# AnnSeidel/genometools

Hardware: AMD Instinct MI355X
Metric: Gbp/s ESA build (suf+lcp+bwt), 3 Gbp DNA, 1/2/4/8 MI355X; bit-exact vs CPU (higher is better)
Workload: dtype u64; 1 GPU; human-like DNA (2% N, 24 seqs, repeats) n=3000000000 seed=43 -suf -lcp -bwt (BASELINE.json configs[2]); parallelism=1 device, pair_suffixes=341032298, tied_suffixes=390540711, refine_rounds=9, maxbranchdepth=8256

## Files before the change

### genometools_amd/csrc/esa_engine.hip

```cpp
#include <stdarg.h>
#include <stdlib.h>
#include <chrono>
#include <type_traits>
#include <utility>
#include <vector>
#include "../../include/gtamd_esa.h"
#include "esa_prims.h"
#include "esa_devutil.h"
#include "esa_own.h"

static thread_local char g_err[1024] = "";
void gtamd_set_error(const char *fmt, ...) {
  va_list ap;
  va_start(ap, fmt);
  vsnprintf(g_err, sizeof g_err, fmt, ap);
  va_end(ap);
}
extern "C" const char *gtamd_esa_last_error(void) { return g_err; }

extern "C" int gtamd_device_count(void) {
  GTAMD_ABI_BEGIN
  int n = 0;
  if (hipGetDeviceCount(&n) != hipSuccess) return 0;
  return n;
// ... 1532 lines not shown
      xfirst[y][x] = (r & PAIR_SWAP) != 0;
    }
    u64 pos[4];
    int who[4] = {0, 0, 0, 0};
    for (int k = 0; k < g; k++) pos[k] = sa[i + k];
    for (int k = 0; k < g; k++) {
      int place = 0;
      for (int o = 0; o < g; o++)
        if (o != k && xfirst[o][k]) place++;
      who[place] = k;
    }
    u32 perm = 0;
    for (int k = 0; k < g; k++) {
      sa[i + k] = (P) pos[who[k]];
      perm |= (u32) who[k] << (2 * k);
      if (k > 0) {
        const u32 lv = lc[who[k - 1]][who[k]];
        slcp[3 * j + (k - 1)] = lv;
        sum += lv;
        nlarge += lv >= GTAMD_LCPOVERFLOW;
        mx = lv > mx ? lv : mx;
      }
    }
    sres[j] = perm | ((u32) g << 8);
    for (int k = 1; k < g; k++) {
      const u64 e = i + k;
      atomicAnd(reinterpret_cast<unsigned long long *>(&tiebits2[e >> 6]), ~(1ull << (e & 63)));
    }
    done = (u32) g;
  }
#pragma unroll
  for (int d = 32; d >= 1; d >>= 1) {
    sum += __shfl_xor(sum, d, 64);
    nlarge += __shfl_xor(nlarge, d, 64);
    done += __shfl_xor(done, d, 64);
    const u32 o = __shfl_xor(mx, d, 64);
    mx = o > mx ? o : mx;
  }
  if (lane == 0) { s_sum[w] = sum; s_large[w] = nlarge; s_max[w] = mx; s_cnt[w] = done; }
  __syncthreads();
  if (threadIdx.x == 0) {
    unsigned long long S = 0, Lg = 0;
    u32 M = 0, D = 0;
    for (int x = 0; x < 4; x++) {
      S += s_sum[x]; Lg += s_large[x]; D += s_cnt[x]; M = s_max[x] > M ? s_max[x] : M;
    }
    if (S) atomicAdd(&stats->lcpsum, S);
    if (Lg) atomicAdd(&stats->numlarge, Lg);
    if (M) atomicMax(&stats->maxlcp, M);
    if (D) atomicAdd(&stats->smalldone, (unsigned long long) D);
  }
}

template <typename P>
__global__ __launch_bounds__(256) void k_small_apply(
    const u32 *__restrict__ sidx, const u32 *__restrict__ sres, const u32 *__restrict__ slcp,
    u64 ns, const P *__restrict__ sa, u64 *__restrict__ suf, u8 *__restrict__ lcp,
    u8 *__restrict__ bwt, u32 *__restrict__ lcpfull, u64 index_offset, Stats *stats) {
  for (u64 j = (u64) blockIdx.x * 256 + threadIdx.x; j < ns; j += (u64) gridDim.x * 256) {
    const u32 r = sres[j];
    const u64 i = sidx[j];
    const int g = (int) (r >> 8) & 7;
    u8 old[4] = {0, 0, 0, 0};
    if (bwt != nullptr)
      for (int k = 0; k < g; k++) old[k] = bwt[i + k];
    for (int k = 0; k < g; k++) {
      const u64 p = sa[i + k];
      if (suf != nullptr) suf[i + k] = p;
      if (bwt != nullptr) bwt[i + k] = old[(r >> (2 * k)) & 3u];
      if (p == 0) stats->longest = index_offset + i + k;
      if (k > 0 && lcp != nullptr) {
        const u32 lv = slcp[3 * j + (k - 1)];
        lcp[i + k] = (u8) (lv < GTAMD_LCPOVERFLOW ? lv : GTAMD_LCPOVERFLOW);
        if (lv >= GTAMD_LCPOVERFLOW) lcpfull[i + k] = lv;
      }
    }
  }
}

constexpr int PE_STAGE = 2048;
template <typename P>
__global__ __launch_bounds__(256) void k_pair_emit(
    const u64 *__restrict__ tiebits, u64 nwords, const u32 *__restrict__ off,
    const P *__restrict__ sa, P *__restrict__ pkey, u64 *__restrict__ pval,
    u32 *__restrict__ pidx) {
  __shared__ u32 s_scan[4];
  __shared__ P s_pk[PE_STAGE];
  __shared__ u64 s_pv[PE_STAGE];
  __shared__ u32 s_pi[PE_STAGE];
  const u64 w = (u64) blockIdx.x * 256 + threadIdx.x;
  u64 ph = 0;
  if (w < nwords) {
    const u64 t = tiebits[w];
    const u64 nx = w + 1 < nwords ? tiebits[w + 1] : 0ull;
    ph = pair_heads(t, nx);
  }
  u32 tot;
  u32 local = block_scan_excl_sum((u32) __popcll(ph), &tot, s_scan);
  const u32 base = off[blockIdx.x];
  const bool staged = tot <= (u32) PE_STAGE;
  while (ph) {
    const int b = __ffsll((unsigned long long) ph) - 1;
    ph &= ph - 1;
    const u64 i = w * 64 + b;
    const u64 j = (u64) base + local;
    const P a = sa[i];
    const u64 v = (sizeof(P) == 4 ? (u64) sa[i + 1] : i) | (j << 32);
    if (staged) { s_pk[local] = a; s_pv[local] = v; s_pi[local] = (u32) i; }
    else { pkey[j] = a; pval[j] = v; pidx[j] = (u32) i; }
    local++;
  }
  if (!staged) return;
  __syncthreads();
  for (u32 k = threadIdx.x; k < tot; k += 256) {
    pkey[base + k] = s_pk[k];
    pval[base + k] = s_pv[k];
    pidx[base + k] = s_pi[k];
  }
}

constexpr int PR_LINE = 16;
template <int BITS, typename P>
__global__ __launch_bounds__(256) void k_pair_resolve(
    Text t, const P *__restrict__ pkey, const u64 *__restrict__ pval, u64 nrec, u64 np,
    const P *__restrict__ sa, u32 *__restrict__ res, Stats *stats, int chunk) {
  __shared__ unsigned long long s_sum[4], s_large[4];
  __shared__ u32 s_max[4];
  const int lane = threadIdx.x & 63, w = threadIdx.x >> 6;
  unsigned long long sum = 0, nlarge = 0;
  u32 mx = 0;
  const u64 nchunks = (nrec + chunk - 1) / chunk;
  for (u64 c = (u64) blockIdx.x * 256 + threadIdx.x; c < nchunks;
       c += (u64) gridDim.x * 256) {
    constexpr int RING = 4;
    u64 ra[RING] = {0, 0, 0, 0}, rb[RING] = {0, 0, 0, 0}, rl[RING] = {0, 0, 0, 0};
    bool rf[RING] = {true, true, true, true};
    int filled = 0;
    for (int e0 = 0; e0 < chunk; e0 += PR_LINE) {
      const u64 s0 = c * chunk + e0;
      if (s0 >= nrec) break;
      P ak[PR_LINE];
      u64 ivk[PR_LINE];
      if (s0 + PR_LINE <= nrec) {
        if (sizeof(P) == 4) {
#pragma unroll
          for (int q = 0; q < PR_LINE / 4; q++) {
            const uint4 v = *reinterpret_cast<const uint4 *>(pkey + s0 + 4 * q);
            ak[4 * q] = (P) v.x; ak[4 * q + 1] = (P) v.y; ak[4 * q + 2] = (P) v.z; ak[4 * q + 3] = (P) v.w;
          }
        } else {
#pragma unroll
          for (int q = 0; q < PR_LINE / 2; q++) {
            const ulonglong2 v = *reinterpret_cast<const ulonglong2 *>(pkey + s0 + 2 * q);
            ak[2 * q] = (P) v.x; ak[2 * q + 1] = (P) v.y;
          }
        }
#pragma unroll
        for (int q = 0; q < PR_LINE / 2; q++) {
          const ulonglong2 v = *reinterpret_cast<const ulonglong2 *>(pval + s0 + 2 * q);
          ivk[2 * q] = v.x; ivk[2 * q + 1] = v.y;
        }
      } else {
#pragma unroll
        for (int q = 0; q < PR_LINE; q++) {
          ak[q] = s0 + q < nrec ? pkey[s0 + q] : (P) 0;
          ivk[q] = s0 + q < nrec ? pval[s0 + q] : 0ull;
        }
      }
#pragma unroll
    for (int e = 0; e < PR_LINE; e++) {
      const u64 s = s0 + e;
      if (s >= nrec || e0 + e >= chunk) continue;
      const u64 a = ak[e];
      const u64 iv = ivk[e];
      const u64 j = iv >> 32;
      const u64 b = sizeof(P) == 4 ? (iv & 0xFFFFFFFFull) : (u64) sa[(iv & 0xFFFFFFFFull) + 1];
      u64 l = 0;
      bool a_first = true, known = false;
#pragma unroll
      for (int k = 0; k < RING; k++) {
        if (k < filled && !known) {
          const u64 d = a - ra[k];
          if (b >= rb[k] && b - rb[k] == d && rl[k] >= (u64) Key<BITS>::KNOWN + d) {
            l = rl[k] - d;
            a_first = rf[k];
            known = true;
          }
        }
      }
      if (!known) l = lcp_extend_long<BITS, 4>(t, a, b, (u64) Key<BITS>::KNOWN, &a_first);
#pragma unroll
      for (int k = RING - 1; k > 0; k--) { ra[k] = ra[k - 1]; rb[k] = rb[k - 1]; rl[k] = rl[k - 1]; rf[k] = rf[k - 1]; }
      ra[0] = a; rb[0] = b; rl[0] = l; rf[0] = a_first;
      if (filled < RING) filled++;
      const u32 lv = l < 0x7FFFFFFFull ? (u32) l : 0x7FFFFFFFu;
      res[j] = lv | (a_first ? 0u : PAIR_SWAP);
      if (j < np) {
        sum += lv;
        nlarge += lv >= GTAMD_LCPOVERFLOW;
        mx = lv > mx ? lv : mx;
      }
    }
    }
  }
#pragma unroll
  for (int d = 32; d >= 1; d >>= 1) {
    sum += __shfl_xor(sum, d, 64);
    nlarge += __shfl_xor(nlarge, d, 64);
    const u32 o = __shfl_xor(mx, d, 64);
    mx = o > mx ? o : mx;
  }
  if (lane == 0) { s_sum[w] = sum; s_large[w] = nlarge; s_max[w] = mx; }
  __syncthreads();
  if (threadIdx.x == 0) {
    unsigned long long S = 0, Lg = 0;
    u32 M = 0;
    for (int i = 0; i < 4; i++) {
      S += s_sum[i]; Lg += s_large[i]; M = s_max[i] > M ? s_max[i] : M;
    }
    if (S) atomicAdd(&stats->lcpsum, S);
    if (Lg) atomicAdd(&stats->numlarge, Lg);
    if (M) atomicMax(&stats->maxlcp, M);
  }
}

__global__ __launch_bounds__(256) void k_pair_swapbits(
    const u64 *__restrict__ tiebits, u64 nwords, const u32 *__restrict__ off,
    const u32 *__restrict__ res, u64 *__restrict__ swp) {
  __shared__ u32 s_scan[4];
  const u64 w = (u64) blockIdx.x * 256 + threadIdx.x;
  u64 t = 0, ph = 0;
  if (w < nwords) {
    t = tiebits[w];
    const u64 nx = w + 1 < nwords ? tiebits[w + 1] : 0ull;
    ph = pair_heads(t, nx);
  }
  u32 tot;
  const u32 j0 = off[blockIdx.x] + block_scan_excl_sum((u32) __popcll(ph), &tot, s_scan);
  if (w >= nwords) return;
  u64 up = 0, down = 0;
  if (w > 0 && (pair_heads(tiebits[w - 1], t) >> 63) && (res[j0 - 1] & PAIR_SWAP)) down = 1;
  u32 j = j0;
  for (u64 h = ph; h; h &= h - 1) {
    const int b = __ffsll((unsigned long long) h) - 1;
    if (res[j++] & PAIR_SWAP) up |= 1ull << b;
  }
  down |= up << 1;
  *reinterpret_cast<ulonglong2 *>(swp + 2 * w) = make_ulonglong2(up, down);
}

template <typename P>
__global__ __launch_bounds__(256) void k_pair_apply(
    const u32 *__restrict__ pidx, const u32 *__restrict__ res, u64 np,
    const P *__restrict__ sa, u64 *__restrict__ suf, u8 *__restrict__ lcp,
    u8 *__restrict__ bwt, u32 *__restrict__ lcpfull, u64 index_offset, Stats *stats) {
  for (u64 j = (u64) blockIdx.x * 256 + threadIdx.x; j < np; j += (u64) gridDim.x * 256) {
    const u64 i = pidx[j];
    const u32 r = res[j], lv = r & ~PAIR_SWAP;
    if (lcp != nullptr) {
      lcp[i + 1] = (u8) (lv < GTAMD_LCPOVERFLOW ? lv : GTAMD_LCPOVERFLOW);
      if (lv >= GTAMD_LCPOVERFLOW) lcpfull[i + 1] = lv;
    }
    if (r & PAIR_SWAP) {
      const u64 x = sa[i], y = sa[i + 1];
      if (x == 0) stats->longest = index_offset + i + 1;
      if (suf != nullptr) { suf[i] = y; suf[i + 1] = x; }
      if (bwt != nullptr) {
        const u8 b0 = bwt[i], b1 = bwt[i + 1];
        bwt[i] = b1;
        bwt[i + 1] = b0;
      }
    }
  }
}

constexpr int RT_TILE = 2048;
constexpr int RT_THREADS = 256;
constexpr int RT_PER = RT_TILE / RT_THREADS;

template <typename P> struct RoundKey {
  static constexpr int KK = sizeof(P) == 8 ? 40 : 32;
  static __device__ __forceinline__ u64 pack(u32 lg, bool open, u64 kk, u32 e) {
    return ((u64) lg << (12 + KK)) | ((u64) open << (11 + KK)) | (kk << 11) | (u64) e;
  }
  static __device__ __forceinline__ bool open(u64 key) { return (key >> (11 + KK)) & 1ull; }
};

template <typename P>
__global__ __launch_bounds__(RT_THREADS) void k_round_tile(
    const u32 *__restrict__ uidx, const P *__restrict__ upos,
    const u32 *__restrict__ ugrp, P *__restrict__ k2, u64 m,
    P *__restrict__ cv, u32 *__restrict__ hv, const u32 *__restrict__ tstart,
    u32 *__restrict__ flagbits, const P *__restrict__ rank, u64 h, u64 n) {
  using RK = RoundKey<P>;
  constexpr bool WIDE = sizeof(P) == 8;
  __shared__ u64 s_key[RT_TILE];
  __shared__ P s_pos[RT_TILE];
  __shared__ u64 s_k2w[WIDE ? RT_TILE : 1];
  __shared__ u16 s_start[RT_TILE + 2];
  __shared__ u32 s_scan[4];
  u32 *s_grp = reinterpret_cast<u32 *>(s_key);
  u32 *s_k2n = s_grp + RT_TILE;
  const int tid = threadIdx.x;
  const u64 tile_first = tstart[blockIdx.x], tile_end = tstart[blockIdx.x + 1];
  for (u64 base = tile_first; base < tile_end; base += RT_TILE) {
  const u32 cnt = (u32) ((tile_end - base) < (u64) RT_TILE ? (tile_end - base) : (u64) RT_TILE);
  const u32 g_first = ugrp[base], g_last = ugrp[base + cnt - 1];
  const bool first_open = base > 0 && ugrp[base - 1] == g_first;
  const bool last_open = base + cnt < m && ugrp[base + cnt] == g_last;
#pragma unroll
  for (int c = 0; c < RT_PER; c++) {
    const u32 e = (u32) c * RT_THREADS + tid;
    P kv = 0;
    if (e < cnt) {
      const P p = upos[base + e];
      s_grp[e] = ugrp[base + e];
      s_pos[e] = p;
      if (rank != nullptr) {
        u64 q = (u64) p + h;
        if (q > n) q = n;
        kv = rank[q];
      } else
        kv = k2[base + e];
    } else {
      s_grp[e] = 0xFFFFFFFFu;
      s_pos[e] = 0;
    }
    if (WIDE) s_k2w[e] = (u64) kv; else s_k2n[e] = (u32) kv;
  }
  __syncthreads();
  u32 gr[RT_PER];
  u64 kr[RT_PER];
  const u32 e0 = (u32) tid * RT_PER;
  u64 kprev = tid > 0 ? (WIDE ? s_k2w[e0 - 1] : (u64) s_k2n[e0 - 1]) : 0ull;
  u32 gprev = tid > 0 ? s_grp[e0 - 1] : 0u;
#pragma unroll
  for (int c = 0; c < RT_PER; c++) {
    gr[c] = s_grp[e0 + c];
    kr[c] = WIDE ? s_k2w[e0 + c] : (u64) s_k2n[e0 + c];
  }
  u32 startflags = 0, nstart = 0;
#pragma unroll
  for (int c = 0; c < RT_PER; c++) {
    const u32 e = e0 + c;
    const bool st = e == 0 || gr[c] != gprev;
    gprev = gr[c];
    startflags |= (u32) st << c;
    nstart += st;
  }
  u32 tot;
  u32 lg = block_scan_excl_sum(nstart, &tot, s_scan);
  u32 nflag = 0;
  int splits = 0;
  u32 openbits = 0;
// ... 1397 lines not shown
}

template <int BITS, bool WIDE>
struct Build {
  using K = Key<BITS>;
  using P = typename std::conditional<WIDE, u64, u32>::type;
  static constexpr u64 RANKREC = 1 + sizeof(P) / 4;
  static constexpr u64 ISA_CHUNK = 1ull << 27;

  gtamd_esa_ctx *const c;
  const Switches &sw;
  u32 want;
  const bool dist;
  const u64 N, n;
  const u32 R;
  const hipStream_t st;
  const bool debug;

  u32 prefixlength = 0;
  bool long_prefix = false, want_suf = false, want_lcp = false, want_bwt = false;
  bool msd = false;
  bool msd_part = false;
  bool fused_pass0 = false;

  int fail = 0;

  u64 NL, index_offset = 0;
  Tiles tl;
  u64 Tn;
  u64 prev_key = 0;
  int has_prev = 0;

  bool pass0_done = false;
  u32 *msd_sa = nullptr, *msd_fval = nullptr;
  u64 *msd_fkey = nullptr, msd_local = 0;
  int nev = 0;
  u64 *skey = nullptr;
  P *sa = nullptr;
  u64 *fkey = nullptr;
  u32 *fval = nullptr;
  u64 *d_suf = nullptr;
  u8 *d_lcp = nullptr, *d_bwt = nullptr;
  bool emitted = false;

  u64 *tiebits = nullptr;
  u64 *tiebits2 = nullptr;
  u64 numties = 0, anyties = 0;
  u64 nwords = 0, nwb = 0;
  u64 m0 = 0;
  u64 m0_tied_all = 0;
  u64 anyleft = 0;
  u64 npairs = 0, nsmall = 0, nrec = 0;
  u64 rank_built = 0;
  u32 rounds = 0;
  int nb = 0, nbl = 0;
  int ps[8], pw[8], pn = 0;

  struct Words {
    u32 *cntw, *headw, *offw, *carry;
    u32 *pcnt, *poff;
    u32 *scnt, *soff;
    u32 *rcnt, *roff;
    u32 *scanws;
    u32 *pws;
    void carve(u32 *base, u64 nw) {
      cntw = base;
      headw = cntw + nw + 16;
      offw = headw + nw + 16;
      carry = offw + nw + 16;
      pcnt = carry + nw + 16;
      poff = pcnt + nw + 16;
      scnt = poff + nw + 16;
      soff = scnt + nw + 16;
      rcnt = soff + nw + 16;
      roff = rcnt + nw + 16;
      scanws = roff + nw + 16;
      pws = scanws + scan_workspace_words(nw) + 64;
    }
  } wd;

  struct PairLists {
    P *pk_a, *pk_b;
    u64 *pv_a, *pv_b;
    u32 *pidx, *pres, *prws, *sidx, *sres, *slcp, *srec;
    u8 *ssize;
    u64 *swp;
    void carve(Bump &a, u64 records, u64 pairs, u64 groups, u64 nw) {
      const u64 pp = (records + 64 + 3) & ~3ull;
      const u64 sp = (groups + 64 + 3) & ~3ull;
      pk_a = a.take<P>(pp); pk_b = a.take<P>(pp);
      pv_a = a.take<u64>(pp); pv_b = a.take<u64>(pp);
      pidx = a.take<u32>(pp); pres = a.take<u32>(pp);
      prws = a.take<u32>(radix_workspace_words(records));
      sidx = a.take<u32>(sp); sres = a.take<u32>(sp); slcp = a.take<u32>(3 * sp);
      srec = a.take<u32>(sp);
      ssize = a.take<u8>(sp);
      swp = a.take<u64>(pairs > 0 ? 2 * nw + 8 : 0);
    }
  } pl;
  const u64 *pair_swp = nullptr;
  int apply_early = 0;
  u64 apply_wgs = 256;
  u32 *lcpfull = nullptr;

  struct Rounds {
    u32 *uidx0, *uidx, *ugrp, *uidx2, *ugrp2;
    P *upos, *upos2;
    P *cvo;
    u32 *hv;
    u64 *keep;
    u32 *koff;
    P *k2;
    u32 *flagbits;
    u32 *tstart;
    P *fk2, *fk2s_a, *fk2s_b, *fpos, *cvs;
    u32 *fgrp, *fj, *perm_a, *perm_b, *gk_a, *gk_b, *fhv;
    P *lk_a, *lk_b;
    u32 *lv_a, *lv_b;
    u32 *rws2, *scanws2;
    u32 *xoff, *xorder, *xqoff, *xmsg, *xbc_q, *xbo_q, *xbc_u, *xbo_u;
    P *xrank, *xans;
    u8 *xdest_q, *xdest_u;
    void carve(Bump &a, u64 mp, u64 tied, u64 items, u32 parts, bool exchange) {
      uidx0 = a.take<u32>(mp); uidx = a.take<u32>(mp); ugrp = a.take<u32>(mp);
      uidx2 = a.take<u32>(mp); ugrp2 = a.take<u32>(mp);
      upos = a.take<P>(mp); upos2 = a.take<P>(mp);
      cvo = a.take<P>(mp);
      hv = a.take<u32>(mp);
      keep = a.take<u64>(mp / 64 + 4);
      koff = a.take<u32>(mp);
      k2 = a.take<P>(mp);
      flagbits = a.take<u32>(mp / 32 + RT_TILE / 32 + 64);
      tstart = a.take<u32>(mp / RT_STRIDE_MIN + 64);
      fk2 = a.take<P>(mp); fk2s_a = a.take<P>(mp); fk2s_b = a.take<P>(mp);
      fpos = a.take<P>(mp); cvs = a.take<P>(mp);
      fgrp = a.take<u32>(mp); fj = a.take<u32>(mp);
      perm_a = a.take<u32>(mp); perm_b = a.take<u32>(mp);
      gk_a = a.take<u32>(mp); gk_b = a.take<u32>(mp);
      fhv = a.take<u32>(mp);
      lk_a = a.take<P>(mp); lk_b = a.take<P>(mp);
      lv_a = a.take<u32>(mp); lv_b = a.take<u32>(mp);
      rws2 = a.take<u32>(radix_workspace_words(tied));
      scanws2 = a.take<u32>(scan_workspace_words(mp > dest_words(parts, items) ? mp : dest_words(parts, items)));
      xoff = xorder = xqoff = xmsg = xbc_q = xbo_q = xbc_u = xbo_u = nullptr;
      xrank = xans = nullptr;
      xdest_q = xdest_u = nullptr;
      if (exchange) {
        xoff = a.take<u32>(items + 64); xorder = a.take<u32>(items + 64);
        xrank = a.take<P>(items + 64); xans = a.take<P>(items + 64);
        xqoff = a.take<u32>(items + 64);
        xmsg = a.take<u32>((items + 64) * (RANKREC + 1));
        xdest_q = a.take<u8>(items + 64); xdest_u = a.take<u8>(items + 64);
        xbc_q = a.take<u32>(dest_words(parts, items)); xbo_q = a.take<u32>(dest_words(parts, items));
        xbc_u = a.take<u32>(dest_words(parts, items)); xbo_u = a.take<u32>(dest_words(parts, items));
      }
    }
  } ar;
  u64 xm = 0;
  u64 xrecv_n = 0;
  u32 *xrecv_msg = nullptr;
  P *xrecv_ans = nullptr;
  P *rank = nullptr;
  P *isa = nullptr;

  struct RankWindows {
    int wb = 0;
    u64 nwin = 0, nww = 0;
    u64 h0 = 0;
    bool windows = false;
    u32 *w_need = nullptr, *w_built = nullptr, *w_sel = nullptr, *w_pref = nullptr,
        *w_list = nullptr;
    std::vector<u32> h_need, h_built, h_all;
    P *lpos = nullptr;
    u32 *lhead = nullptr;
    u64 list_cap = 0;
  } rk;

  struct RankTable {
    u32 *rank32, *heads, *ppos, *phead, *qhead, *qpos;
    const u32 *spos;
    bool heads_array;
    int wmax, pb, wb, split;
    int fb;
    GroupHeadValues headgen;
  } rt;

  Build(gtamd_esa_ctx *ctx, const Switches &switches, u32 want_, bool dist_)
      : c(ctx), sw(switches), want(want_), dist(dist_), N(ctx->N), n(ctx->n), R(ctx->numparts),
        st(ctx->st), debug(switches.debug), NL(ctx->N), Tn(ctx->N) {
    tl.T = N;
    tl.self = c->part;
  }

  int run() {
    TRY(plan());
    if (!dist) TRY(first_sort_whole());
    else if (msd_part) TRY(first_sort_filtered());
    else TRY(first_sort_exchanged());
    TRY(finish_first_sort());
    TRY(count_ties());
    if (anyties > 0) {
      TRY(count_tied_words());
      bool settled = false;
      TRY(settle_few_ties(&settled));
      if (!settled) {
        TRY(pair_path());
        TRY(place_apply());
        if (apply_early == 1) TRY(apply_beside());
        TRY(count_left());
        TRY(carve_rounds());
        TRY(settle_few_left());
        if (anyleft > 0 && !dist) {
          TRY(prepare_rank_table());
          TRY(build_rank(true));
        }
        if (anyleft > 0 && dist) {
          TRY(prepare_rank_exchange());
          TRY(send_ranks());
        }
        TRY(launch_emission());
        if (apply_early == 2) TRY(apply_beside());
        TRY(doubling_rounds());
        TRY(tie_fix());
      }
    }
    return report();
  }

  int fork_second_stream() {
    HIP_TRY(hipEventRecord(c->ev_sorted, st));
    HIP_TRY(hipStreamWaitEvent(c->st2, c->ev_sorted, 0));
    return 0;
  }

  int launch_emission() {
    if (emitted) return 0;
    emitted = true;
    TRY(fork_second_stream());
    if (NL > 0) {
      k_finalize<BITS, P><<<stride_grid(div_up(NL, FIN_TILE)), FIN_THREADS, 0, c->st2>>>(
          skey, sa, NL, prefixlength, d_suf, d_lcp, d_bwt, nullptr,
          c->d_stats, prev_key, has_prev, index_offset);
      HIP_TRY(hipGetLastError());
    }
    HIP_TRY(hipEventRecord(c->ev_emitted, c->st2));
    return 0;
  }

  int tie_words(const u64 *bits) {
    if (NL > 0) {
      k_tie_words<<<(u32) nwb, 256, 0, st>>>(bits, nwords, wd.cntw, wd.headw);
      HIP_TRY(hipGetLastError());
      TRY(scan_u32(SCAN_SUM, wd.cntw, wd.offw, nwb, false, wd.scanws, st));
      TRY(scan_u32(SCAN_MAX, wd.headw, wd.carry, nwords, false, wd.scanws, st));
    }
    k_total<<<1, 1, 0, st>>>(wd.offw, wd.cntw, NL > 0 ? nwb : 0, c->d_stats);
    HIP_TRY(hipGetLastError());
    TRY(fetch_stats(c));
    return 0;
  }

  u64 direct_limit() const { return NL / 512 > 4096 ? NL / 512 : 4096; }
  int direct_ties(const u32 *uidx0, const u32 *ugrp, bool clear_fallback) {
    TRY(launch_emission());
    HIP_TRY(hipStreamWaitEvent(st, c->ev_emitted, 0));
    if (clear_fallback) HIP_TRY(hipMemsetAsync(&c->d_stats->dfallback, 0, 4, st));
    if (m0 > 0) {
      k_direct_ties<BITS, P><<<(u32) div_up(m0, 256), 256, 0, st>>>(
          c->text, uidx0, ugrp, m0, sa, d_suf, d_lcp, d_bwt, want_lcp,
          index_offset, c->d_stats);
      HIP_TRY(hipGetLastError());
    }
    TRY(fetch_stats(c));
    return 0;
  }
  int drop_direct_stats() {
    HIP_TRY(hipMemsetAsync(&c->d_stats->dsum, 0, 8, st));
    HIP_TRY(hipMemsetAsync(&c->d_stats->dmax, 0, 4, st));
    return 0;
  }

  int plan() {
    prefixlength = c->user_prefixlength ? c->user_prefixlength
                                        : gtamd_recommended_prefixlength(c->sigma, n);
    long_prefix = prefixlength > (u32) K::SYMS;
    if (long_prefix && (want & GTAMD_WANT_LCP)) want |= GTAMD_WANT_SUF;
    want_suf = want & GTAMD_WANT_SUF;
    want_lcp = want & GTAMD_WANT_LCP;
    want_bwt = want & GTAMD_WANT_BWT;
    if (dist && (want & GTAMD_WANT_BCK)) {
      gtamd_set_error("the bucket table is not available from a part build");
      return -1;
    }
    if (R > 1 && (c->comm_allgather == nullptr || c->comm_alltoallv == nullptr)) {
      gtamd_set_error("a part build needs the collective callbacks "
                      "(gtamd_esa_set_comm)");
      return -1;
    }
    memset(&c->timing, 0, sizeof c->timing);
    memset(&c->stats, 0, sizeof c->stats);
    c->alloc_ms = 0;
    c->llv_pairs = 0;
    if (!dist && !WIDE && !(want & GTAMD_WANT_BCK) && N >= 64 && (BITS == 2 || (prefixlength <= 9 && c->sigma <= 20))) {
      msd = sw.msd >= 0 ? sw.msd == 1 : N >= (1ull << 25);
    }
    if (dist && BITS == 2) msd_part = !sw.msd_part_off;
    fused_pass0 = !dist && !msd && BITS == 2 && sw.fused_pass0;
    if (debug)
      fprintf(stderr, "gtamd: part %u: run: parts=%u positions=%d first_sort=%s pass0=%s\n", c->part, R,
              WIDE ? 64 : 32, msd || msd_part ? "msd" : "lsd",
              dist || msd || BITS != 2 ? "none" : (fused_pass0 ? "fused" : "plain"));
    return 0;
  }

  int first_sort_whole() {
    TRY(ensure_workspace(c, N, want, false));
    HIP_TRY(hipMemsetAsync(c->d_stats, 0, sizeof(Stats), st));
    HIP_TRY(hipEventRecord(c->ev[EV_START], st));
    if (msd) {
      TRY(msd_sort_emit<BITS == 5 ? 1 : 0>(c, sw, want, prefixlength, N, N, nullptr, &msd_sa, &msd_fkey, &msd_fval,
                                           &msd_local));
      HIP_TRY(hipEventRecord(c->ev_emitted, st));
    } else if (fused_pass0) {
      const u32 ntiles = (u32) div_up(N, KP_TILE);
      k_dc_hist_dna<<<ntiles, KP_THREADS, 0, st>>>(c->text, N, c->rws.as<u32>());
      HIP_TRY(hipGetLastError());
      TRY(radix_scan_tile_hist(c->rws.as<u32>(), N, st));
      k_keygen_pass0_dna<<<ntiles, KP_THREADS, 0, st>>>(c->text, N, c->rws.as<u32>(),
                                                      c->k1.as<u64>(), c->v1.as<u32>());
      pass0_done = true;
    } else if (BITS == 2)
      k_keygen_dna<<<(u32) div_up(N, 1024), 256, 0, st>>>(c->text, 0, N, c->k0.as<u64>(),
                                                          c->v0.as<u32>());
    else
      k_keygen<BITS><<<(u32) div_up(N, 1024), 256, 0, st>>>(c->text, 0, N, c->k0.as<u64>(),
                                                            c->v0.as<u32>());
    HIP_TRY(hipGetLastError());
    return 0;
  }

  int first_sort_filtered() {
    msd = true;
    tl.T = Tiles::size_for(N, R);
    Tn = tl.count(c->part, N);
    fail = filter_and_sort() != 0;
    HIP_TRY(hipEventRecord(c->ev_emitted, st));
    return 0;
  }
// ... 250 lines not shown
  }

  int count_tied_words() {
    nwords = div_up(NL, 64);
    nwb = div_up(nwords, 256);
    wd.carve(c->rws.as<u32>(), nwords);
    TRY(tie_words(tiebits));
    m0 = c->h_stats->count;
    return 0;
  }

  int settle_few_ties(bool *settled) {
    *settled = false;
    u64 small = m0 <= direct_limit();
    if (R > 1) TRY(allgather_word(c, 0, RED_AND, &small));
    if (!small) return 0;
    const u64 mp = (m0 + 64 + 3) & ~3ull;
    const int bad = ensure_buf(c, c->arena, mp * (12 + sizeof(P)) + 4096, "the tied suffixes") != 0;
    if (!bad) {
      Bump a = {c->arena.as<u8>(), 0};
      u32 *uidx0 = a.take<u32>(mp), *uidx = a.take<u32>(mp), *ugrp = a.take<u32>(mp);
      P *upos = a.take<P>(mp);
      if (m0 > 0) {
        k_unres_emit<P><<<(u32) div_up(nwords, 256), 256, 0, st>>>(
            tiebits, nwords, wd.offw, wd.carry, sa, uidx0, uidx, upos, ugrp);
        HIP_TRY(hipGetLastError());
      }
      TRY(direct_ties(uidx0, ugrp, false));
    }
    u64 gaveup = bad ? 1 : c->h_stats->dfallback;
    if (R > 1) TRY(allgather_word(c, bad, RED_OR, &gaveup));
    else if (bad) return -1;
    *settled = gaveup == 0;
    if (!*settled) TRY(drop_direct_stats());
    return 0;
  }

  int pair_path() {
    TRY(ensure_buf(c, c->tiebits2, (nwords + 2) * 8, "the tie bitmap"));
    tiebits2 = c->tiebits2.as<u64>();
    const bool no_pairs = sw.no_pairs;
    const bool no_small = no_pairs || sw.no_small_groups;
    u64 nsrec = 0;
    if (NL > 0) {
      if (no_pairs) {
        HIP_TRY(hipMemcpyAsync(tiebits2, tiebits, nwords * 8, hipMemcpyDeviceToDevice, st));
      } else {
        k_pair_words<<<(u32) nwb, 256, 0, st>>>(tiebits, nwords, wd.pcnt, wd.scnt, wd.rcnt, tiebits2);
        HIP_TRY(hipGetLastError());
        TRY(scan_u32(SCAN_SUM, wd.pcnt, wd.poff, nwb, false, wd.scanws, st));
        TRY(scan_u32(SCAN_SUM, wd.scnt, wd.soff, nwb, false, wd.scanws, st));
        TRY(scan_u32(SCAN_SUM, wd.rcnt, wd.roff, nwb, false, wd.scanws, st));
        k_total2<<<1, 1, 0, st>>>(wd.poff, wd.pcnt, nwb, c->d_stats);
        k_total3<<<1, 1, 0, st>>>(wd.soff, wd.scnt, nwb, c->d_stats);
        k_total<<<1, 1, 0, st>>>(wd.roff, wd.rcnt, nwb, c->d_stats);
        HIP_TRY(hipGetLastError());
        TRY(fetch_stats(c));
        npairs = c->h_stats->count2;
        nsmall = c->h_stats->count3;
        nsrec = c->h_stats->count;
      }
    }
    if (no_small || nsrec > NL / 8 || npairs + nsrec >= SINGLE_LIMIT) { nsmall = 0; nsrec = 0; }
    nrec = npairs + nsrec;
    apply_early = sw.apply_early;
    {
      Bump sz = {nullptr, 0};
      pl.carve(sz, nrec, npairs, nsmall, nwords);
      fail = ensure_buf(c, c->arena_p, sz.off + 4096, "the pairs of tied suffixes") != 0;
      if (!fail && want_lcp && apply_early && nrec > 0)
        fail = ensure_buf(c, c->lcpfull_buf, (NL + 8) * 4, "the LCP values beyond the byte") != 0;
      if (R > 1) TRY(comm_allgather(c, fail, nullptr, nullptr, 0));
      else if (fail) return -1;
      Bump a = {c->arena_p.as<u8>(), 0};
      pl.carve(a, nrec, npairs, nsmall, nwords);
    }
    nb = bits_for(N - 1);
    nbl = bits_for(NL ? NL - 1 : 0);
    pn = passes_for(0, nb, ps, pw);
    pair_swp = npairs > 0 ? pl.swp : nullptr;
    if (nrec == 0) return 0;
    if (npairs > 0) {
      k_pair_emit<P><<<(u32) div_up(nwords, 256), 256, 0, st>>>(tiebits, nwords, wd.poff, sa, pl.pk_a,
                                                               pl.pv_a, pl.pidx);
      HIP_TRY(hipGetLastError());
    }
    if (nsmall > 0) {
      k_small_emit<P><<<(u32) div_up(nwords, 256), 256, 0, st>>>(
          tiebits, nwords, wd.soff, wd.roff, sa, npairs, pl.sidx, pl.ssize, pl.srec, pl.pk_a, pl.pv_a);
      HIP_TRY(hipGetLastError());
    }
    TRY(radix_sort_pairs<P, u64>(pl.pk_a, pl.pv_a, pl.pk_b, pl.pv_b, nrec, ps, pw, pn, pl.prws, st,
                                 nullptr, nullptr));
    const P *pk_sorted = (pn & 1) ? pl.pk_b : pl.pk_a;
    const u64 *pv_sorted = (pn & 1) ? pl.pv_b : pl.pv_a;
    TRY(launch_emission());
    int pair_chunk = (int) (nrec >> 20 < 16 ? 16 : (nrec >> 20 > 128 ? 128 : nrec >> 20));
    if (sw.pair_chunk > 0) pair_chunk = sw.pair_chunk;
    pair_chunk = (pair_chunk + PR_LINE - 1) / PR_LINE * PR_LINE;
    if (debug)
      fprintf(stderr, "gtamd: part %u: pair resolve: records=%llu chunk=%d grid=%u\n", c->part,
              (unsigned long long) nrec, pair_chunk,
              stride_grid(div_up(div_up(nrec, (u64) pair_chunk), 256)));
    k_pair_resolve<BITS, P><<<stride_grid(div_up(div_up(nrec, (u64) pair_chunk), 256)), 256, 0, st>>>(
        c->text, pk_sorted, pv_sorted, nrec, npairs, sa, pl.pres, c->d_stats, pair_chunk);
    HIP_TRY(hipGetLastError());
    if (npairs > 0) {
      k_pair_swapbits<<<(u32) nwb, 256, 0, st>>>(tiebits, nwords, wd.poff, pl.pres, pl.swp);
      HIP_TRY(hipGetLastError());
    }
    if (nsmall > 0) {
      k_small_combine<P><<<(u32) div_up(nsmall, 256), 256, 0, st>>>(
          pl.sidx, pl.ssize, pl.srec, pl.pres, nsmall, sa, tiebits2, pl.sres, pl.slcp, c->d_stats);
      HIP_TRY(hipGetLastError());
    }
    return 0;
  }

  int place_apply() {
    if (want_lcp && apply_early && nrec > 0) lcpfull = c->lcpfull_buf.as<u32>();
    if (nrec == 0) apply_early = 0;
    int cus = 0;
    if (hipDeviceGetAttribute(&cus, hipDeviceAttributeMultiprocessorCount, c->device) == hipSuccess && cus > 0)
      apply_wgs = (u64) cus;
    if (sw.apply_wgs > 0) apply_wgs = sw.apply_wgs;
    return 0;
  }
  int launch_apply(hipStream_t s) {
    u64 cap = ~0ull;
    if (apply_early == 1) cap = apply_wgs;
    else if (apply_early == 2 && m0 > 0) {
      cap = apply_wgs;
      if (!sw.apply_wgs_given) {
        const double need = 7.7e-8 * (double) npairs + 2.85e-7 * (double) nsmall;
        const double have = 1.25 * 4.0e-7 * (double) m0 + 0.5;
        if (need > have) cap = (u64) ((double) apply_wgs * (need / have));
      }
    }
    if (debug) {
      const u64 gpair = div_up(npairs, 256), gsmall = div_up(nsmall, 256);
      fprintf(stderr, "gtamd: part %u: apply: placement=%d pair_grid=%llu small_grid=%llu\n", c->part,
              apply_early, (unsigned long long) (gpair < cap ? gpair : cap),
              (unsigned long long) (gsmall < cap ? gsmall : cap));
    }
    if (npairs > 0) {
      const u64 g = div_up(npairs, 256);
      k_pair_apply<P><<<(u32) (g < cap ? g : cap), 256, 0, s>>>(
          pl.pidx, pl.pres, npairs, sa, d_suf, d_lcp, d_bwt, lcpfull, index_offset, c->d_stats);
      HIP_TRY(hipGetLastError());
    }
    if (nsmall > 0) {
      const u64 g = div_up(nsmall, 256);
      k_small_apply<P><<<(u32) (g < cap ? g : cap), 256, 0, s>>>(
          pl.sidx, pl.sres, pl.slcp, nsmall, sa, d_suf, d_lcp, d_bwt, lcpfull, index_offset, c->d_stats);
      HIP_TRY(hipGetLastError());
    }
    return 0;
  }
  int apply_beside() {
    TRY(fork_second_stream());
    TRY(launch_apply(c->st2));
    HIP_TRY(hipEventRecord(c->ev_applied, c->st2));
    return 0;
  }

  int count_left() {
    TRY(tie_words(tiebits2));
    m0 = c->h_stats->count;
    const u64 smalldone = c->h_stats->smalldone;
    anyleft = m0;
    if (R > 1) TRY(allgather_word(c, 0, RED_SUM, &anyleft));
    if (debug)
      fprintf(stderr, "gtamd: part %u: %llu tied with a neighbour, %llu pairs, %llu small groups "
              "(%llu entries settled), %llu left\n",
              c->part, (unsigned long long) numties, (unsigned long long) npairs,
              (unsigned long long) nsmall, (unsigned long long) smalldone,
              (unsigned long long) m0);
    return 0;
  }

  int carve_rounds() {
    const u64 mp = (m0 + 64 + 3) & ~3ull;
    const u64 ichunk = NL < ISA_CHUNK ? NL : ISA_CHUNK;
    xm = dist ? (ichunk > mp ? ichunk : mp) : 0;
    xrecv_n = (u64) R * ISA_CHUNK > anyleft ? (u64) R * ISA_CHUNK : anyleft;
    if (xrecv_n > Tn) xrecv_n = Tn;
    xrecv_n += 64;
    {
      Bump sz = {nullptr, 0};
      ar.carve(sz, mp, m0, xm, R, dist);
      fail = ensure_buf(c, c->arena, sz.off + 4096, "the refinement of tied suffixes") != 0;
      if (dist && !fail)
        fail = ensure_buf(c, c->xrecv, xrecv_n * (8 + 2 * sizeof(P)) + 1024,
                          "the exchange of ranks") != 0;
      if (dist && !fail)
        fail = ensure_buf(c, c->winbuf, (3 * (div_up(N, 1ull << 16) / 32 + 2) + 16) * 4,
                          "the rank windows") != 0;
      if (R > 1) TRY(comm_allgather(c, fail, nullptr, nullptr, 0));
      else if (fail) return -1;
      Bump a = {c->arena.as<u8>(), 0};
      ar.carve(a, mp, m0, xm, R, dist);
    }
    xrecv_msg = c->xrecv.as<u32>();
    xrecv_ans = reinterpret_cast<P *>(c->xrecv.as<u8>() + ((xrecv_n * (4 + 4 * RANKREC) + 255) & ~255ull));
    if (m0 > 0) {
      k_unres_emit<P><<<(u32) div_up(nwords, 256), 256, 0, st>>>(
          tiebits2, nwords, wd.offw, wd.carry, sa, ar.uidx0, ar.uidx, ar.upos, ar.ugrp);
      HIP_TRY(hipGetLastError());
    }
    return 0;
  }

  int settle_few_left() {
    m0_tied_all = m0;
    if (dist || m0 == 0 || m0 > direct_limit()) return 0;
    TRY(direct_ties(ar.uidx0, ar.ugrp, true));
    if (c->h_stats->dfallback == 0) {
      m0 = 0;
      anyleft = 0;
    } else {
      TRY(drop_direct_stats());
    }
    return 0;
  }

  int prepare_rank_table() {
    TRY(ensure_buf(c, c->isa_tmp, (NL + 8) * 8, "the rank table build"));
    rt.rank32 = fval;
    rank = reinterpret_cast<P *>(rt.rank32);
    rt.heads = reinterpret_cast<u32 *>(fkey);
    rt.ppos = c->isa_tmp.as<u32>(); rt.phead = rt.ppos + ((NL + 3) & ~3ull);
    rt.qhead = rt.heads; rt.qpos = rt.heads + ((NL + 3) & ~3ull);
    rt.wmax = sw.rank_window_bits;
    rt.spos = reinterpret_cast<const u32 *>(sa);
    rt.heads_array = bits_for(N - 1) <= rt.wmax;
    rt.pb = nb > rt.wmax ? nb - rt.wmax : 0;
    if (rt.pb > 16) rt.pb = 16;
    rt.wb = nb - rt.pb;
    if (rt.wb > rt.wmax + 1) {
      gtamd_set_error("rank table: %d position bits do not fit two passes and a "
                      "%d-bit window", nb, rt.wmax);
      return -1;
    }
    rt.split = rt.wb > rt.wmax ? 2 : 1;
    rt.fb = rt.wmax < RW_FINE ? rt.wmax : RW_FINE;
// ... 402 lines not shown
    HIP_TRY(hipGetLastError());
    TRY(fetch_stats(c));
    const u64 nf = c->h_stats->count;
    if (debug)
      fprintf(stderr, "gtamd: part %u round %u: %llu entries in groups across tile borders "
              "(%u tiles, stride %u)\n", c->part, rounds, (unsigned long long) nf, ntiles, rt_stride);
    if (nf > 0) {
      k_flag_gather<P><<<nfb, RT_THREADS, 0, st>>>(ar.flagbits, tileoff, ar.ugrp, ar.k2, ar.upos, m, ar.fk2,
                                                     ar.fk2s_a, ar.fgrp, ar.fpos, ar.fj, ar.perm_a);
      HIP_TRY(hipGetLastError());
      TRY(radix_sort_pairs<P, u32>(ar.fk2s_a, ar.perm_a, ar.fk2s_b, ar.perm_b, nf, ps, pw, pn, ar.rws2, st,
                                   nullptr, nullptr));
      u32 *perm1 = (pn & 1) ? ar.perm_b : ar.perm_a, *permx = (pn & 1) ? ar.perm_a : ar.perm_b;
      const u32 gf = (u32) div_up(nf, 256);
      k_gather_u32<<<gf, 256, 0, st>>>(ar.fgrp, perm1, nf, ar.gk_a);
      HIP_TRY(hipGetLastError());
      TRY(radix_sort_pairs<u32, u32>(ar.gk_a, perm1, ar.gk_b, permx, nf, s.gs, s.gw, s.gn, ar.rws2, st,
                                     nullptr, nullptr));
      const u32 *perm2 = (s.gn & 1) ? permx : perm1;
      k_flag_heads<P><<<gf, 256, 0, st>>>(perm2, ar.fgrp, ar.fk2, ar.fpos, ar.uidx, ar.fj, nf, ar.fhv, ar.cvs);
      HIP_TRY(hipGetLastError());
      TRY(scan_u32(SCAN_MAX, ar.fhv, ar.fhv, nf, true, ar.scanws2, st));
      k_flag_scatter<P><<<gf, 256, 0, st>>>(ar.cvs, ar.fhv, ar.fj, nf, ar.cvo, ar.hv);
      HIP_TRY(hipGetLastError());
    }
    u32 *bcnt = ar.koff, *boffs = ar.koff + g + 16;
    k_round_apply<P><<<g, 256, 0, st>>>(ar.cvo, ar.hv, ar.uidx, ar.ugrp, m, index_offset, sa,
                                        dist ? nullptr : rank, ar.keep, bcnt);
    HIP_TRY(hipGetLastError());
    TRY(scan_u32(SCAN_SUM, bcnt, boffs, g, false, ar.scanws2, st));
    k_round_compact<P><<<g, 256, 0, st>>>(ar.keep, boffs, bcnt, ar.uidx, ar.cvo, ar.hv, m, ar.uidx2,
                                          ar.upos2, ar.ugrp2, c->d_stats);
    HIP_TRY(hipGetLastError());
    TRY(fetch_stats(c));
    s.m = c->h_stats->count;
    s.h *= 2;
    if (dist) {
      s.ru.cval = ar.cvo; s.ru.gnew = ar.hv; s.ru.ugrp = ar.ugrp; s.ru.index_offset = index_offset;
      s.ru.tl = tl; s.ru.isa = isa; s.ru.soff = ar.xoff; s.ru.srank = ar.xrank;
      s.m_upd = m;
      TRY(dest_count(c, s.ru, s.m_upd, ar.xdest_u, ar.xbc_u, ar.xbo_u, ar.scanws2, 1));
      s.rq.upos = ar.upos2; s.rq.h = s.h;
      TRY(dest_count(c, s.rq, s.m, ar.xdest_q, ar.xbc_q, ar.xbo_q, ar.scanws2, 0));
    }
    std::swap(ar.uidx, ar.uidx2);
    std::swap(ar.ugrp, ar.ugrp2);
    std::swap(ar.upos, ar.upos2);
    if (dist) s.ru.ugrp = ar.ugrp2;
    return 0;
  }

  int tie_fix() {
    TRY(launch_emission());
    HIP_TRY(hipStreamWaitEvent(st, c->ev_emitted, 0));
    if (want_lcp && !apply_early) {
      if (!dist) lcpfull = fval;
      else if (WIDE) lcpfull = fval;
      else lcpfull = c->isa_tmp.as<u32>();
    }
    if (!apply_early) TRY(launch_apply(st));
    const u32 g0 = (u32) div_up(m0, 256);
    u32 *bcnt0 = ar.koff, *boff0 = ar.koff + g0 + 16;
    if (m0 > 0) {
      TRY(fork_second_stream());
      k_fix_basic<BITS, P><<<g0, 256, 0, c->st2>>>(c->text, ar.uidx0, m0, sa, d_suf, d_bwt,
                                                   c->d_stats, index_offset);
      HIP_TRY(hipGetLastError());
      HIP_TRY(hipEventRecord(c->ev_emitted, c->st2));
    }
    if (want_lcp && m0 > 0) {
      k_tied_counts<<<g0, 256, 0, st>>>(ar.uidx0, m0, tiebits2, bcnt0);
      HIP_TRY(hipGetLastError());
      TRY(scan_u32(SCAN_SUM, bcnt0, boff0, g0, false, ar.scanws2, st));
      k_total<<<1, 1, 0, st>>>(boff0, bcnt0, g0, c->d_stats);
      HIP_TRY(hipGetLastError());
      TRY(fetch_stats(c));
      const u64 m1 = c->h_stats->count;
      k_lcp_pairs<P><<<g0, 256, 0, st>>>(boff0, tiebits2, ar.uidx0, sa, m0, ar.lk_a, ar.lv_a);
      HIP_TRY(hipGetLastError());
      TRY(radix_sort_pairs<P, u32>(ar.lk_a, ar.lv_a, ar.lk_b, ar.lv_b, m1, ps, pw, pn, ar.rws2, st,
                                   nullptr, nullptr));
      const P *pk = (pn & 1) ? ar.lk_b : ar.lk_a;
      const u32 *pv = (pn & 1) ? ar.lv_b : ar.lv_a;
      k_lcp_chunks<BITS, P><<<stride_grid(div_up(div_up(m1, LCP_CHUNK), 256)), 256, 0, st>>>(
          c->text, pk, pv, m1, sa, d_lcp, lcpfull, c->d_stats);
      HIP_TRY(hipGetLastError());
    }
    if (apply_early) HIP_TRY(hipStreamWaitEvent(st, c->ev_applied, 0));
    if (!want_lcp) return 0;
    TRY(fetch_stats(c));
    const u64 pairs = c->h_stats->numlarge;
    if (pairs * 16 > c->llv.bytes) HIP_TRY(c->llv.alloc((pairs + pairs / 4 + 1024) * 16));
    if (pairs > 0) {
      const u32 gl = (u32) div_up(NL, LLV_TILE);
      u32 *lc = wd.cntw, *lo = wd.offw;
      k_large_counts<<<gl, 256, 0, st>>>(d_lcp, NL, lc);
      HIP_TRY(hipGetLastError());
      TRY(scan_u32(SCAN_SUM, lc, lo, gl, false, wd.scanws, st));
      k_llv_emit<<<gl, 256, 0, st>>>(d_lcp, NL, lcpfull, lo, index_offset, c->llv);
      HIP_TRY(hipGetLastError());
    }
    c->llv_pairs = pairs;
    return 0;
  }

  int report() {
    TRY(launch_emission());
    HIP_TRY(hipStreamWaitEvent(st, c->ev_emitted, 0));
    HIP_TRY(hipEventRecord(c->ev[EV_DONE], st));
    TRY(fetch_stats(c));

    c->stats.totallength = n;
    c->stats.numberofallsortedsuffixes = N;
    c->stats.longest = c->h_stats->longest;
    c->stats.largelcpvalues = want_lcp ? c->h_stats->numlarge : 0;
    c->stats.maxbranchdepth =
        want_lcp ? (c->h_stats->maxlcp > c->h_stats->dmax ? c->h_stats->maxlcp
                                                           : c->h_stats->dmax) : 0;
    c->stats.lcptabsum = want_lcp ? c->h_stats->lcpsum + c->h_stats->dsum : 0;
    if (long_prefix && want_lcp) {
      HIP_TRY(hipMemsetAsync(&c->d_stats->msum, 0, 8, st));
      if (c->NL > 0) {
        k_masked_lcpsum<<<stride_grid(div_up(c->NL, 256)), 256, 0, st>>>(
            c->text, c->suf.as<u64>(), c->lcp.as<u8>(), c->NL, prefixlength, c->d_stats);
        HIP_TRY(hipGetLastError());
      }
      if (c->llv_pairs > 0) {
        k_masked_llvsum<<<stride_grid(div_up(c->llv_pairs, 256)), 256, 0, st>>>(
            c->text, c->suf.as<u64>(), c->llv, c->llv_pairs, c->index_offset, prefixlength,
            c->d_stats);
        HIP_TRY(hipGetLastError());
      }
      TRY(fetch_stats(c));
      c->stats.lcptabsum = c->h_stats->msum;
    }
    c->stats.prefixlength = prefixlength;
    c->stats.refine_rounds = rounds;
    c->stats.tied_suffixes = (m0_tied_all ? m0_tied_all : m0) + 2 * npairs + c->h_stats->smalldone;
    c->stats.pair_suffixes = 2 * npairs;
    c->stats.device_bytes = c->alloc_bytes;
    float ms = 0;
    HIP_TRY(hipEventElapsedTime(&ms, c->ev[EV_START], c->ev[EV_DONE])); c->timing.total_ms = ms;
    HIP_TRY(hipEventElapsedTime(&ms, c->ev[EV_START], c->ev[EV_KEYS])); c->timing.keygen_ms = ms;
    HIP_TRY(hipEventElapsedTime(&ms, c->ev[EV_KEYS], c->ev[EV_SORTED])); c->timing.sort_ms = ms;
    HIP_TRY(hipEventElapsedTime(&ms, c->ev[EV_SORTED], c->ev[EV_TIEBITS])); c->timing.finalize_ms = ms;
    HIP_TRY(hipEventElapsedTime(&ms, c->ev[EV_REFINE_BEGIN], c->ev[EV_REFINE_END])); c->timing.refine_ms = ms;
    HIP_TRY(hipEventElapsedTime(&ms, c->ev[EV_REFINE_END], c->ev[EV_DONE])); c->timing.tie_fix_ms = ms;
    float sc = 0;
    for (int i = 0; i < nev; i++) {
      HIP_TRY(hipEventElapsedTime(&ms, c->ev_scatter[2 * i], c->ev_scatter[2 * i + 1]));
      sc += ms;
    }
    if (msd && msd_local > 0) {
      HIP_TRY(hipEventElapsedTime(&sc, c->ev_scatter[0], c->ev_scatter[1]));
      nev = 1;
    }
    c->timing.scatter_ms = sc;
    c->timing.scatter_launches = (u32) nev;
    c->timing.scatter_items = msd ? msd_local : NL;
    c->timing.scatter_read_items = c->timing.scatter_items;
    c->timing.scatter_written_items = msd ? msd_local - c->h_stats->crowded : NL;
    c->stats.msd_crowded_entries = msd ? c->h_stats->crowded : 0;
    c->stats.rank_entries_built = rank_built;
    c->timing.dominant_kernel = msd ? 1u : 0u;
    c->timing.alloc_ms = c->alloc_ms;
    c->want = want;
    c->ran = true;
    return 0;
  }
};

// ... 165 lines not shown
```

Baseline: 26.49 Gbp/s.

## Apply pair results via tiebit tiles with shared-memory lcp/bwt staging

```diff
diff --git a/genometools_amd/csrc/esa_engine.hip b/genometools_amd/csrc/esa_engine.hip
--- a/genometools_amd/csrc/esa_engine.hip
+++ b/genometools_amd/csrc/esa_engine.hip
@@ -1638,12 +1638,10 @@
 template <typename P>
 __global__ __launch_bounds__(256) void k_pair_emit(
     const u64 *__restrict__ tiebits, u64 nwords, const u32 *__restrict__ off,
-    const P *__restrict__ sa, P *__restrict__ pkey, u64 *__restrict__ pval,
-    u32 *__restrict__ pidx) {
+    const P *__restrict__ sa, P *__restrict__ pkey, u64 *__restrict__ pval) {
   __shared__ u32 s_scan[4];
   __shared__ P s_pk[PE_STAGE];
   __shared__ u64 s_pv[PE_STAGE];
-  __shared__ u32 s_pi[PE_STAGE];
   const u64 w = (u64) blockIdx.x * 256 + threadIdx.x;
   u64 ph = 0;
   if (w < nwords) {
@@ -1662,8 +1660,8 @@
     const u64 j = (u64) base + local;
     const P a = sa[i];
     const u64 v = (sizeof(P) == 4 ? (u64) sa[i + 1] : i) | (j << 32);
-    if (staged) { s_pk[local] = a; s_pv[local] = v; s_pi[local] = (u32) i; }
-    else { pkey[j] = a; pval[j] = v; pidx[j] = (u32) i; }
+    if (staged) { s_pk[local] = a; s_pv[local] = v; }
+    else { pkey[j] = a; pval[j] = v; }
     local++;
   }
   if (!staged) return;
@@ -1671,7 +1669,6 @@
   for (u32 k = threadIdx.x; k < tot; k += 256) {
     pkey[base + k] = s_pk[k];
     pval[base + k] = s_pv[k];
-    pidx[base + k] = s_pi[k];
   }
 }
 
@@ -1806,26 +1803,140 @@
 }
 
 template <typename P>
-__global__ __launch_bounds__(256) void k_pair_apply(
-    const u32 *__restrict__ pidx, const u32 *__restrict__ res, u64 np,
-    const P *__restrict__ sa, u64 *__restrict__ suf, u8 *__restrict__ lcp,
-    u8 *__restrict__ bwt, u32 *__restrict__ lcpfull, u64 index_offset, Stats *stats) {
-  for (u64 j = (u64) blockIdx.x * 256 + threadIdx.x; j < np; j += (u64) gridDim.x * 256) {
-    const u64 i = pidx[j];
-    const u32 r = res[j], lv = r & ~PAIR_SWAP;
-    if (lcp != nullptr) {
-      lcp[i + 1] = (u8) (lv < GTAMD_LCPOVERFLOW ? lv : GTAMD_LCPOVERFLOW);
-      if (lv >= GTAMD_LCPOVERFLOW) lcpfull[i + 1] = lv;
-    }
-    if (r & PAIR_SWAP) {
-      const u64 x = sa[i], y = sa[i + 1];
-      if (x == 0) stats->longest = index_offset + i + 1;
-      if (suf != nullptr) { suf[i] = y; suf[i + 1] = x; }
-      if (bwt != nullptr) {
-        const u8 b0 = bwt[i], b1 = bwt[i + 1];
-        bwt[i] = b1;
-        bwt[i + 1] = b0;
-      }
+__device__ __forceinline__ void pair_suf_entries(
+    u64 i, const P *__restrict__ sa, u64 *__restrict__ suf, u64 index_offset, Stats *stats) {
+  const u64 x = sa[i], y = sa[i + 1];
+  if (x == 0) stats->longest = index_offset + i + 1;
+  if (suf != nullptr) { suf[i] = y; suf[i + 1] = x; }
+}
+
+constexpr int PT_WORDS = 256;
+constexpr int PT_ENTRIES = PT_WORDS * 64;
+constexpr int PT_VECS = PT_ENTRIES / 16 / 256;
+constexpr int PT_RES = 4;
+
+__device__ __forceinline__ void tile_load(const u8 *__restrict__ tab, u64 base, u64 N,
+                                          uint4 (&r)[PT_VECS]) {
+#pragma unroll
+  for (int q = 0; q < PT_VECS; q++) {
+    const u64 o = base + (u64) (q * 256 + threadIdx.x) * 16;
+    if (o + 16 <= N) r[q] = *reinterpret_cast<const uint4 *>(tab + o);
+    else {
+      u32 v[4] = {0, 0, 0, 0};
+      for (int k = 0; k < 16; k++)
+        if (o + k < N) v[k >> 2] |= (u32) tab[o + k] << (8 * (k & 3));
+      r[q] = make_uint4(v[0], v[1], v[2], v[3]);
+    }
+  }
+}
+__device__ __forceinline__ void tile_store(u8 *__restrict__ tab, u64 base, u64 N,
+                                           const uint4 *__restrict__ s_tab) {
+#pragma unroll
+  for (int q = 0; q < PT_VECS; q++) {
+    const u64 o = base + (u64) (q * 256 + threadIdx.x) * 16;
+    if (o + 16 <= N) *reinterpret_cast<uint4 *>(tab + o) = s_tab[q * 256 + threadIdx.x];
+    else {
+      const u8 *sb = reinterpret_cast<const u8 *>(s_tab + q * 256 + threadIdx.x);
+      for (int k = 0; k < 16; k++)
+        if (o + k < N) tab[o + k] = sb[k];
+    }
+  }
+}
+
+template <typename P>
+__global__ __launch_bounds__(256) void k_pair_apply_tiles(
+    const u64 *__restrict__ tiebits, u64 nwords, const u32 *__restrict__ off,
+    const u32 *__restrict__ res, u64 N, const P *__restrict__ sa, u64 *__restrict__ suf,
+    u8 *__restrict__ lcp, u8 *__restrict__ bwt, u32 *__restrict__ lcpfull, u64 index_offset,
+    Stats *stats) {
+  __shared__ u32 s_scan[4];
+  __shared__ uint4 s_lcp[PT_ENTRIES / 16], s_bwt[PT_ENTRIES / 16];
+  u8 *const bl = reinterpret_cast<u8 *>(s_lcp), *const bb = reinterpret_cast<u8 *>(s_bwt);
+  const u64 ntiles = (nwords + PT_WORDS - 1) / PT_WORDS;
+  u64 tile = blockIdx.x;
+  if (tile >= ntiles) return;
+  uint4 rl[PT_VECS], rb[PT_VECS];
+  u64 t = 0, nx = 0;
+  {
+    const u64 w = tile * PT_WORDS + threadIdx.x;
+    if (w < nwords) t = tiebits[w];
+    if (w + 1 < nwords) nx = tiebits[w + 1];
+    if (lcp != nullptr) tile_load(lcp, tile * PT_ENTRIES, N, rl);
+    if (bwt != nullptr) tile_load(bwt, tile * PT_ENTRIES, N, rb);
+  }
+  for (;;) {
+    const u64 base = tile * PT_ENTRIES;
+#pragma unroll
+    for (int q = 0; q < PT_VECS; q++) {
+      if (lcp != nullptr) s_lcp[q * 256 + threadIdx.x] = rl[q];
+      if (bwt != nullptr) s_bwt[q * 256 + threadIdx.x] = rb[q];
+    }
+    u64 ph = pair_heads(t, nx);
+    u32 tot;
+    const u32 j0 = off[tile] + block_scan_excl_sum((u32) __popcll(ph), &tot, s_scan);
+    if (threadIdx.x == PT_WORDS - 1) ph &= ~(1ull << 63);
+    const int cnt = __popcll(ph);
+    u32 rv[PT_RES];
+#pragma unroll
+    for (int k = 0; k < PT_RES; k++) rv[k] = k < cnt ? res[j0 + k] : 0u;
+    const u64 next = tile + gridDim.x;
+    if (next < ntiles) {
+      const u64 w = next * PT_WORDS + threadIdx.x;
+      t = w < nwords ? tiebits[w] : 0ull;
+      nx = w + 1 < nwords ? tiebits[w + 1] : 0ull;
+      if (lcp != nullptr) tile_load(lcp, next * PT_ENTRIES, N, rl);
+      if (bwt != nullptr) tile_load(bwt, next * PT_ENTRIES, N, rb);
+    }
+    int k = 0;
+    for (u64 h = ph; h; h &= h - 1, k++) {
+      const u32 e = threadIdx.x * 64 + (u32) (__ffsll((unsigned long long) h) - 1);
+      u32 r = k == 0 ? rv[0] : k == 1 ? rv[1] : k == 2 ? rv[2] : rv[3];
+      if (k >= PT_RES) r = res[j0 + k];
+      const u32 lv = r & ~PAIR_SWAP;
+      if (lcp != nullptr) {
+        bl[e + 1] = (u8) (lv < GTAMD_LCPOVERFLOW ? lv : GTAMD_LCPOVERFLOW);
+        if (lcpfull != nullptr && lv >= GTAMD_LCPOVERFLOW) lcpfull[base + e + 1] = lv;
+      }
+      if (r & PAIR_SWAP) {
+        pair_suf_entries<P>(base + e, sa, suf, index_offset, stats);
+        if (bwt != nullptr) {
+          const u8 b0 = bb[e], b1 = bb[e + 1];
+          bb[e] = b1;
+          bb[e + 1] = b0;
+        }
+      }
+    }
+    __syncthreads();
+    if (lcp != nullptr) tile_store(lcp, base, N, s_lcp);
+    if (bwt != nullptr) tile_store(bwt, base, N, s_bwt);
+    if (next >= ntiles) break;
+    tile = next;
+    __syncthreads();
+  }
+}
+
+template <typename P>
+__global__ __launch_bounds__(256) void k_pair_apply_borders(
+    const u64 *__restrict__ tiebits, u64 nwords, const u32 *__restrict__ off,
+    const u32 *__restrict__ res, const P *__restrict__ sa, u64 *__restrict__ suf,
+    u8 *__restrict__ lcp, u8 *__restrict__ bwt, u32 *__restrict__ lcpfull, u64 index_offset,
+    Stats *stats) {
+  const u64 b = (u64) blockIdx.x * 256 + threadIdx.x + 1;
+  const u64 w = b * PT_WORDS - 1;
+  if (w + 1 >= nwords) return;
+  if (!(pair_heads(tiebits[w], tiebits[w + 1]) >> 63)) return;
+  const u64 i = w * 64 + 63;
+  const u32 r = res[off[b] - 1], lv = r & ~PAIR_SWAP;
+  if (lcp != nullptr) {
+    lcp[i + 1] = (u8) (lv < GTAMD_LCPOVERFLOW ? lv : GTAMD_LCPOVERFLOW);
+    if (lcpfull != nullptr && lv >= GTAMD_LCPOVERFLOW) lcpfull[i + 1] = lv;
+  }
+  if (r & PAIR_SWAP) {
+    pair_suf_entries<P>(i, sa, suf, index_offset, stats);
+    if (bwt != nullptr) {
+      const u8 b0 = bwt[i], b1 = bwt[i + 1];
+      bwt[i] = b1;
+      bwt[i + 1] = b0;
     }
   }
 }
@@ -3389,7 +3500,7 @@
   struct PairLists {
     P *pk_a, *pk_b;
     u64 *pv_a, *pv_b;
-    u32 *pidx, *pres, *prws, *sidx, *sres, *slcp, *srec;
+    u32 *pres, *prws, *sidx, *sres, *slcp, *srec;
     u8 *ssize;
     u64 *swp;
     void carve(Bump &a, u64 records, u64 pairs, u64 groups, u64 nw) {
@@ -3397,7 +3508,7 @@
       const u64 sp = (groups + 64 + 3) & ~3ull;
       pk_a = a.take<P>(pp); pk_b = a.take<P>(pp);
       pv_a = a.take<u64>(pp); pv_b = a.take<u64>(pp);
-      pidx = a.take<u32>(pp); pres = a.take<u32>(pp);
+      pres = a.take<u32>(pp);
       prws = a.take<u32>(radix_workspace_words(records));
       sidx = a.take<u32>(sp); sres = a.take<u32>(sp); slcp = a.take<u32>(3 * sp);
       srec = a.take<u32>(sp);
@@ -3408,6 +3519,7 @@
   const u64 *pair_swp = nullptr;
   int apply_early = 0;
   u64 apply_wgs = 256;
+  bool apply_forked = false, apply_joined = false;
   u32 *lcpfull = nullptr;
 
   struct Rounds {
@@ -3571,6 +3683,7 @@
   int direct_ties(const u32 *uidx0, const u32 *ugrp, bool clear_fallback) {
     TRY(launch_emission());
     HIP_TRY(hipStreamWaitEvent(st, c->ev_emitted, 0));
+    TRY(join_apply());
     if (clear_fallback) HIP_TRY(hipMemsetAsync(&c->d_stats->dfallback, 0, 4, st));
     if (m0 > 0) {
       k_direct_ties<BITS, P><<<(u32) div_up(m0, 256), 256, 0, st>>>(
@@ -3987,7 +4100,7 @@
     if (nrec == 0) return 0;
     if (npairs > 0) {
       k_pair_emit<P><<<(u32) div_up(nwords, 256), 256, 0, st>>>(tiebits, nwords, wd.poff, sa, pl.pk_a,
-                                                               pl.pv_a, pl.pidx);
+                                                               pl.pv_a);
       HIP_TRY(hipGetLastError());
     }
     if (nsmall > 0) {
@@ -4042,17 +4155,22 @@
         if (need > have) cap = (u64) ((double) apply_wgs * (need / have));
       }
     }
-    if (debug) {
-      const u64 gpair = div_up(npairs, 256), gsmall = div_up(nsmall, 256);
+    const u64 gpair = npairs > 0 ? nwb : 0, gsmall = div_up(nsmall, 256);
+    if (debug)
       fprintf(stderr, "gtamd: part %u: apply: placement=%d pair_grid=%llu small_grid=%llu\n", c->part,
               apply_early, (unsigned long long) (gpair < cap ? gpair : cap),
               (unsigned long long) (gsmall < cap ? gsmall : cap));
-    }
     if (npairs > 0) {
-      const u64 g = div_up(npairs, 256);
-      k_pair_apply<P><<<(u32) (g < cap ? g : cap), 256, 0, s>>>(
-          pl.pidx, pl.pres, npairs, sa, d_suf, d_lcp, d_bwt, lcpfull, index_offset, c->d_stats);
+      k_pair_apply_tiles<P><<<(u32) (gpair < cap ? gpair : cap), 256, 0, s>>>(
+          tiebits, nwords, wd.poff, pl.pres, NL, sa, d_suf, d_lcp, d_bwt, lcpfull, index_offset,
+          c->d_stats);
       HIP_TRY(hipGetLastError());
+      if (nwb > 1) {
+        k_pair_apply_borders<P><<<(u32) div_up(nwb - 1, 256), 256, 0, s>>>(
+            tiebits, nwords, wd.poff, pl.pres, sa, d_suf, d_lcp, d_bwt, lcpfull, index_offset,
+            c->d_stats);
+        HIP_TRY(hipGetLastError());
+      }
     }
     if (nsmall > 0) {
       const u64 g = div_up(nsmall, 256);
@@ -4066,6 +4184,12 @@
     TRY(fork_second_stream());
     TRY(launch_apply(c->st2));
     HIP_TRY(hipEventRecord(c->ev_applied, c->st2));
+    apply_forked = true;
+    return 0;
+  }
+  int join_apply() {
+    if (apply_forked && !apply_joined) HIP_TRY(hipStreamWaitEvent(st, c->ev_applied, 0));
+    apply_joined = true;
     return 0;
   }
 
@@ -4634,11 +4758,12 @@
                                    nullptr, nullptr));
       const P *pk = (pn & 1) ? ar.lk_b : ar.lk_a;
       const u32 *pv = (pn & 1) ? ar.lv_b : ar.lv_a;
+      TRY(join_apply());
       k_lcp_chunks<BITS, P><<<stride_grid(div_up(div_up(m1, LCP_CHUNK), 256)), 256, 0, st>>>(
           c->text, pk, pv, m1, sa, d_lcp, lcpfull, c->d_stats);
       HIP_TRY(hipGetLastError());
     }
-    if (apply_early) HIP_TRY(hipStreamWaitEvent(st, c->ev_applied, 0));
+    TRY(join_apply());
     if (!want_lcp) return 0;
     TRY(fetch_stats(c));
     const u64 pairs = c->h_stats->numlarge;
```

Result: no change. 26.34 Gbp/s, median of 2 (-0.6%).
